# dongzhuoyao/self-guided-diffusion-models

Hardware: AMD Instinct MI355X
Metric: cfg_sampled_images_per_sec_64x64_1000step_ddpm (higher is better)
Workload: dtype f32 as 3xf16 split MFMA products, f32 accumulate; 1 GPU; IN64 unet_fast ch128 cluster-k5000 cond_scale=2 bs=40/GPU (UNet batch 80), 1000-step native DDPM; batch_per_gpu=40, unet_batch=80, precision_mode=f16x3, launch=hipGraph-captured step

## Files before the change

### include/sgdm_hip.h

```cpp
#ifndef SGDM_HIP_H
#define SGDM_HIP_H
#include <stdint.h>

#ifdef __cplusplus
extern "C" {
#endif

#define SGD_ABI_VERSION 24
int sgd_abi_version(void);
const char* sgd_build_id(void);

enum { SGD_MODE_FLAT = 0, SGD_MODE_CONV3 = 1 };
enum { SGD_RS_NONE = 0, SGD_RS_AVGPOOL2 = 1, SGD_RS_UP2 = 2,
       SGD_RS_ZEROUP2 = 3 ,
       SGD_RS_UP2_SUBPIXEL = 4 };
enum { SGD_PRO_NONE = 0, SGD_PRO_AFFINE_NC = 1, SGD_PRO_LN_ROW = 2 };
enum { SGD_PREC_F32 = 0, SGD_PREC_F16X3 = 1, SGD_PREC_BF16X3 = 2, SGD_PREC_F16 = 3, SGD_PREC_BF16 = 4 };

typedef struct sgd_igemm_args {
    const float* x0;
    const float* x1;
    int32_t c0, c1;
    int32_t mode;
    int32_t n, hi, wi;
// ... 21 lines not shown
    uint32_t drop_seed;
    float* stats;
    const float* w_scale_inv;
    void* work;
    int64_t work_bytes;
    int32_t grid_cap;
    int32_t tune;
} sgd_igemm_args;
enum {
    SGD_TUNE_BN128 = 1,
    SGD_TUNE_BN256 = 2,
    SGD_TUNE_FLAT2 = 4,
    SGD_TUNE_DEFER = 8,
    SGD_TUNE_PLAIN_SCHEDULE = 16,
    SGD_TUNE_NO_SMALL = 64,
    SGD_TUNE_LN_PACKED = 32,
    SGD_TUNE_WGRAD_GENERIC_NARROW = 256,
    SGD_TUNE_WGRAD_NO_POOLED_PLANES = 512,
    SGD_TUNE_WGRAD_F32 = 1024,
    SGD_TUNE_WGRAD_NO_WS = 2048,
    SGD_TUNE_WGRAD_NO_PLANES = 4096,
    SGD_TUNE_WGRAD_NO_PIPE = 8192,
    SGD_TUNE_WGRAD_PLANES_ALWAYS = 16384,
    SGD_TUNE_NO_SUBPIXEL = 32768
};
int64_t sgd_igemm_work_bytes(void);
int64_t sgd_igemm_work_status_offset(void);
int sgd_igemm_tail_layout(int32_t total_tiles, int32_t nchunks, int32_t taps, int32_t grid, int32_t* out);


int sgd_igemm(const sgd_igemm_args* args , void* stream);
int sgd_igemm_stats_parts(const sgd_igemm_args* args );
int sgd_igemm_subpixel_ok(const sgd_igemm_args* args );

int64_t sgd_packed_weight_bytes(int32_t cout, int32_t cin, int32_t ksize, int32_t prec);
int sgd_pack_weight(const float* w_src, void* w_dst, int32_t cout, int32_t cin, int32_t ksize,
                    int32_t prec, int32_t* cin_p, int32_t* cout_p , void* stream);

int64_t sgd_packed_weight_subpixel_bytes(int32_t cout, int32_t cin, int32_t prec);
int sgd_weight_amax_subpixel(const float* w_src, int32_t cout, int32_t cin, uint32_t* amax_bits, void* stream);
int sgd_pack_weight_subpixel_scaled(const float* w_src, void* w_dst, int32_t cout, int32_t cin, int32_t prec,
                                    const uint32_t* amax_bits, float* scale_inv_out, int32_t* cin_p, int32_t* cout_p ,
                                    void* stream);

int sgd_weight_amax(const float* w, int64_t count, uint32_t* amax_bits, void* stream);
int sgd_pack_weight_scaled(const float* w_src, void* w_dst, int32_t cout, int32_t cin, int32_t ksize, int32_t prec,
                           int32_t transpose ,
                           const uint32_t* amax_bits, float* scale_inv_out, int32_t* cin_p, int32_t* cout_p ,
// ... 228 lines not shown
```

### self-guided-diffusion-models_amd/csrc/igemm.hip

```cpp
#include <type_traits>
#include <utility>

#include "igemm_shared.h"
#include "prologue.h"

namespace {

#ifdef SGDM_PROBE
#define DBG(bit) 0
#define SYNC() do { if (g.stamp) { const unsigned long long t0_ = __builtin_amdgcn_s_memtime(); __syncthreads(); \
                    const unsigned long long t1_ = __builtin_amdgcn_s_memtime(); \
                    if (g.trace && blockIdx.x < 16 && pr_nbar < 512 && (threadIdx.x & 63) == 0) { \
                        unsigned long long* tp_ = g.trace + (((size_t)blockIdx.x * (NTHREADS / 64) + (threadIdx.x >> 6)) * 512 + pr_nbar) * 2; \
                        tp_[0] = t0_; tp_[1] = t1_; } \
                    pr_bar += t1_ - t0_; ++pr_nbar; } else if (!DBG(64)) { __syncthreads(); } } while (0)
#define PROBE_BEGIN() unsigned long long pr_bar = 0, pr_nbar = 0, pr_epi = 0; const unsigned long long pr_t0 = __builtin_amdgcn_s_memtime()
#define PROBE_END(role) do { if (g.stamp && (threadIdx.x & 63) == 0) { \
        unsigned long long* sp_ = g.stamp + ((size_t)blockIdx.x * (NTHREADS / 64) + (threadIdx.x >> 6)) * 4; \
        sp_[0] = __builtin_amdgcn_s_memtime() - pr_t0; sp_[1] = pr_bar; sp_[2] = pr_nbar; sp_[3] = pr_epi; } } while (0)
#define PROBE_EPI(expr) do { if (g.stamp) { const unsigned long long t0_ = __builtin_amdgcn_s_memtime(); expr; pr_epi += __builtin_amdgcn_s_memtime() - t0_; } else { expr; } } while (0)
#else
#define DBG(bit) 0
#define SYNC() __syncthreads()
#define PROBE_BEGIN()
// ... 248 lines not shown
    static constexpr int NA = 3;
    static constexpr int WM = (BN >= 128) ? 128 : 32;
    static constexpr int WN = (BN >= 128) ? BN / 4 : 32;
    static constexpr int MT = WM / 32, NT = WN / 32;
    static constexpr int WAVES_N = BN / WN;
    typedef Frag<PREC, NT> FragT;
    static constexpr bool M16 = PREC != SGD_PREC_F32 && BN <= 128 && !DEFER;
    static constexpr int RB = M16 ? WM / 16 : MT, RBH = M16 ? 16 : 32;
    static constexpr int CBN = M16 ? WN / 16 : NT, CBW = M16 ? 16 : 32;
    static constexpr int QPB = M16 ? 1 : 4;
    typedef Frag16<PREC, CBN> Frag16T;
    typedef std::conditional_t<M16, f32x4, f32x16> AccV;
    static constexpr int NKS = FragT::NKS;

    static constexpr int STG_LD = BN + 4;
    static_assert(!DEFER || (BN == 128 && TAPS == 9 && VEC && !M16), "loader-side epilogue: 3x3, 128-column tiles");
    static_assert(!SUBPIX || (VEC && PREC != SGD_PREC_F32 && BN >= 128), "sub-pixel conv: 16-byte inputs, split modes, 128-column tiles");

    const sgd_igemm_args& a;
    const Geo& g;
    float* As;
    int2* pixtab;
    float* bias_s;
    float* stg;
    int a_floats;
    bool bias_lds;
    int tid, lane, wave;
    int total, xchunk, nloc, xcd, loc, xbeg, xend, cin, nchunks, xtiles, nfull, xrem, split;
    int ntiles, rem_lin, rem_part, last_c0, last_c1;
    int Q, S, s, TW, TH, M;

    __device__ __forceinline__ int lin_of(int k) const { return (rem_lin >= 0 && k == ntiles - 1) ? rem_lin : xbeg + loc + k * nloc; }
    __device__ __forceinline__ int cbeg(int k) const { return k == ntiles - 1 ? last_c0 : 0; }
    __device__ __forceinline__ int cend(int k) const { return k == ntiles - 1 ? last_c1 : nchunks; }

    __device__ __forceinline__ bool init(float* smem) {
        a_floats = g.pix * LDA;
        As = smem;
        pixtab = reinterpret_cast<int2*>(smem + (size_t)NA * a_floats);
        bias_s = smem + (size_t)NA * a_floats + (size_t)g.pix * 8;
        bias_lds = a.cout_p <= BIAS_LDS_MAX;
        stg = bias_s + a.cout_p;

        tid = threadIdx.x; lane = tid & 63;
        wave = __builtin_amdgcn_readfirstlane(tid >> 6);

        total = g.mt * g.nt;
        xchunk = (total + 7) >> 3;
        nloc = gridDim.x >> 3;
// ... 70 lines not shown
        int px = l5;
        if (CONV && g.tw_l2 == 4 && s == 1) {
            if (l5 < 4) px = l5;
            else if (l5 < 12) px = l5 + 4;
            else if (l5 < 16) px = l5 - 8;
            else if (l5 < 20) px = l5;
            else if (l5 < 28) px = l5 + 2;
            else px = l5 < 30 ? l5 - 8 : l5;
        }
        if constexpr (M16) {
            const int i16 = ln & 15;
            px = i16 < 4 ? 2 * i16 : (i16 < 12 ? 2 * (i16 - 4) + 1 : 2 * i16 - 16);
        }
        return px;
    }
    template <int RES, bool PART>
    __device__ __forceinline__ void epilogue(const AccV (&acc)[RB][CBN], const Tile& T, int wm, int wn, int lane_e, int cb, float wsk,
                                             const char* part_base, int nparts) const;
    __device__ __forceinline__ void loader_role();
    __device__ __forceinline__ void compute_role();
};

template <int BN, int PREC, bool VEC, int TAPS, bool DEFER>
__device__ __forceinline__ void IgemmBlock<BN, PREC, VEC, TAPS, DEFER>::loader_role() {
    PROBE_BEGIN();
    __builtin_amdgcn_s_setprio(2);
    const int dlt = tid - NCOMP;
    const int dcq = (dlt >> 6) * 8 + (dlt & 7), drg = (dlt & 63) >> 3;
    int dk = 0, dqs = 0, dnck = cend(0) - cbeg(0);
    Tile dT = tile_at<SUBPIX>(g, lin_of(0), BN, TW, TH);
    int dcol = 0;
    unsigned dsoff = 0xFFFFFFFFu;
    f32x4 dres[8], ds1 = {0.f, 0.f, 0.f, 0.f}, ds2 = ds1;
// ... 67 lines not shown
            const Tile& T = dT;
#pragma unroll
            for (int jj = 0; jj < NQ; ++jj) {
                const int i = i0 + jj;
                const int row = drg + 8 * (i < 16 ? i : 15);
                const int tx = row & (TW - 1), ty = (row >> g.tw_l2) & (TH - 1), nb = row >> (g.tw_l2 + g.th_l2);
                const int n = T.img0 + nb;
                const bool ok = i < i1 && nb < g.nb && n < a.n && dcol < a.cout;
                const int orow = (n * a.ho + T.ty0 + ty) * a.wo + T.tx0 + tx;
                dyoff[jj] = ok ? (unsigned)(((long)orow * a.y_ld + dcol) * 4) : 0xFFFFFFFFu;
                const unsigned ro = ok ? (unsigned)(((long)orow * a.cout + dcol) * 4) : 0xFFFFFFFFu;
                dres[jj] = __builtin_bit_cast(f32x4, __builtin_amdgcn_raw_buffer_load_b128(dr_rs, ro, 0, 0));
            }
        }
        (void)q;
    };
    if constexpr (CONV) {
        const bool uni_rt = VEC && g.nb == 1 && a.pro == SGD_PRO_AFFINE_NC;
        const bool drop_rt = a.drop_p > 0.f;
        const bool lean2 = g.fast_a && VEC && ((uni_rt && a.pro_silu) || (a.pro == SGD_PRO_NONE && !a.pro_silu))
                           && (!drop_rt || (uni_rt && a.pro_silu && a.resample != SGD_RS_AVGPOOL2))
                           && cin % KC == 0 && (a.c1 == 0 || a.c0 % KC == 0) && !DBG(3);
        if (lean2) {
            constexpr int LT = A_THREADS;
            constexpr int AJ = (FAST_PIX * 8 + LT - 1) / LT;
            const int lt = tid - NCOMP;
            const int c4 = lt & 7;
            const int items = g.pix * 8;
            auto go = [&](auto unic, auto poolc, auto dropc) __attribute__((always_inline)) {
                constexpr bool uni = decltype(unic)::value;
// ... 95 lines not shown
#pragma unroll
                    for (int j = 0; j < AJ; ++j) issue_item(s2, j);
                };
                s2.k = 0; s2.chunk = cbeg(0); s2.img0 = tile_at<SUBPIX>(g, lin_of(0), BN, TW, TH).img0; fill(s2);
                load_rows(0);
                issue_coef(s2);
#pragma unroll
                for (int j = 0; j < AJ; ++j) issue_item(s2, j);
                stage(0);
                stage(1);
                SYNC();
                auto periods = [&](auto nqc) __attribute__((always_inline)) {
                    for (int q = 0; q < Q; ++q) {
                        drain(q, nqc);
                        stage((q + 2) % NA);
                        if (q + 4 < Q && (q + 4) % nchunks == 0) build_pixtab((q + 4) / nchunks, lt, LT);
                        SYNC();
                    }
                };
                if constexpr (NS == 4) periods(std::integral_constant<int, 0>());
                else with_nq(periods);
            };
            if (uni_rt) {
                if (a.resample == SGD_RS_AVGPOOL2) go(std::true_type(), std::true_type(), std::false_type());
                else if (drop_rt) go(std::true_type(), std::false_type(), std::true_type());
                else go(std::true_type(), std::false_type(), std::false_type());
            } else {
                if (a.resample == SGD_RS_AVGPOOL2) go(std::false_type(), std::true_type(), std::false_type());
                else go(std::false_type(), std::false_type(), std::false_type());
            }
            PROBE_END(1);
            return;
        }
// ... 235 lines not shown
                tr.tab = cx.tab;
                tr.m0 = 0;
#pragma unroll
                for (int j = 0; j < AJ; ++j)
                    finish_item(slot, tr, cx.chunk, lt + j * A_THREADS, araw[j], kshared, kq);
                cx = ctx_of(qnext);
                request();
            };
            request();
            stage(1, 2);
            SYNC();
            with_nq([&](auto nqc) __attribute__((always_inline)) {
                for (int q = 0; q < Q; ++q) {
                    drain(q, nqc);
                    stage(q + 2, q + 3);
                    if (q + 4 < Q && (q + 4) % nchunks == 0) build_pixtab((q + 4) / nchunks, lt, A_THREADS);
                    SYNC();
                }
            });
        } else {
            stage_A_sync(1, 1);
            SYNC();
            with_nq([&](auto nqc) __attribute__((always_inline)) {
                for (int q = 0; q < Q; ++q) {
                    drain(q, nqc);
                    stage_A_sync(q + 2, q + 2);
                    if (q + 4 < Q && (q + 4) % nchunks == 0) build_pixtab((q + 4) / nchunks, lt, A_THREADS);
                    SYNC();
                }
            });
        }
        PROBE_END(1);
        return;
    } else {
        constexpr int AJ = (BM * 8 + A_THREADS - 1) / A_THREADS;
        f32x4 araw[NB_RING][AJ];
        stage_A_sync(0, 0);
        if (Q > 1) stage_A_sync(1, 1);
        auto issue = [&](int q, auto rc) {
            constexpr int R = decltype(rc)::value;
            q = q < Q ? q : Q - 1;
            const int k = q / nchunks, chunk = q - k * nchunks + cbeg(k);
            const TabRef tab = tabref(k);
            const int c = chunk * KC + c4 * 4;
// ... 28 lines not shown
        for (; step + 3 <= S; step += 3) {
            body(step, R2());
            body(step + 1, R0());
            body(step + 2, R1());
        }
        if (step < S) {
            body(step, R2());
            if (step + 1 < S) body(step + 1, R0());
        }
        PROBE_END(1);
        return;
    }
}

template <int BN, int PREC, bool VEC, int TAPS, bool DEFER>
template <int RES, bool PART>
__device__ __forceinline__ void IgemmBlock<BN, PREC, VEC, TAPS, DEFER>::epilogue(const AccV (&acc)[RB][CBN], const Tile& T, int wm, int wn,
                                                                                 int lane_e, int cb, float wsk, const char* part_base,
                                                                                 int nparts) const {
    const int li = lane & 31;
    bool okm[RB];
    int orw[RB], rrw[RB];
    const int plie = pixel_of_lane(lane_e);
#pragma unroll
    for (int mt = 0; mt < RB; ++mt) {
        const int row = wm * WM + mt * RBH + plie;
        int orow, n = 0, oy = 0, ox = 0;
        if (CONV) {
            const int tx = row & (TW - 1), ty = (row >> g.tw_l2) & (TH - 1), nb = row >> (g.tw_l2 + g.th_l2);
            n = T.img0 + nb; oy = T.ty0 + ty; ox = T.tx0 + tx;
            okm[mt] = nb < g.nb && n < a.n;
// ... 18 lines not shown
    if (vec) {
        float* sp = nullptr;
        if (a.stats) {
            int n_img, part;
            if (CONV) {
                n_img = T.img0;
                part = ((T.par * g.tiles_y + (T.ty0 >> g.th_l2)) * g.tiles_x + (T.tx0 >> g.tw_l2)) * (BM / WM) + wm;
            } else {
                n_img = (int)(T.m0 / a.rows_per_n);
                part = (int)((T.m0 % a.rows_per_n) / BM) * (BM / WM) + wm;
            }
            sp = a.stats + ((long)n_img * g.sparts + part) * 2 * a.cout;
        }
        {
            constexpr int CS = CBN * QPB;
            constexpr int QB = M16 ? ((RES == 2 || PART) ? 1 : (CBN > 2 ? 2 : CBN)) : ((RES == 2 || NT > 1) ? 1 : 2);
            constexpr int RBB = M16 ? (RES == 2 || RB < 4 ? 2 : ((PART || CBN > 2) ? 4 : RB)) : RB;
            static_assert(RB % RBB == 0 && CS % QB == 0, "batches must tile the wave's rows and columns");
#pragma unroll
            for (int q0 = 0; q0 < CS; q0 += QB) {
            f32x4 s1[QB], s2[QB];
#pragma unroll
            for (int i = 0; i < QB; ++i) s1[i] = s2[i] = f32x4{0.f, 0.f, 0.f, 0.f};
#pragma unroll
            for (int mb0 = 0; mb0 < RB; mb0 += RBB) {
#pragma unroll
            for (int mt = mb0; mt < mb0 + RBB; ++mt) asm volatile("" : "+v"(orw[mt]), "+v"(rrw[mt]));
            f32x4 rv[QB][RBB];
            f32x4 pv[QB][RBB];
            if constexpr (PART) {
#pragma unroll
                for (int cs = q0; cs < q0 + QB; ++cs)
#pragma unroll
                    for (int mt = mb0; mt < mb0 + RBB; ++mt) {
                        const char* pp = part_base + (size_t)((mt * CS + cs) * NCOMP) * 16;
// ... 59 lines not shown
            }
        }
    } else {
#pragma unroll
        for (int mt = 0; mt < RB; ++mt) {
            if (!okm[mt]) continue;
            float* yp = a.y + (long)orw[mt] * a.y_ld;
            const float* rp = RES ? a.res + (long)rrw[mt] * a.cout : nullptr;
#pragma unroll
            for (int nt = 0; nt < CBN; ++nt)
#pragma unroll
                for (int gq = 0; gq < QPB; ++gq)
#pragma unroll
                    for (int j = 0; j < 4; ++j) {
                        const int c = cb + nt * CBW + gq * 8 + j;
                        if (c >= a.cout) continue;
                        float x = acc[mt][nt][(M16 ? 0 : gq * 4) + j];
                        if constexpr (PART) {
                            const float* pp = reinterpret_cast<const float*>(part_base + (size_t)(((mt * CBN + nt) * QPB + gq) * NCOMP) * 16) + j;
                            for (int pi = 0; pi < nparts; ++pi) x += pp[pi * (SLAB / 4)];
                        }
                        x = x * wsk + (bias_lds ? bias_s[c] : (a.bias ? a.bias[c] : 0.f));
                        if (RES == 1 || RES == 3) x += rp[c];
                        if (RES == 2) {
                            const long rw = (long)a.wo * 2 * a.cout;
                            x += 0.25f * (rp[c] + rp[a.cout + c] + rp[rw + c] + rp[rw + a.cout + c]);
                        }
                        yp[c] = x;
                    }
        }
// ... 88 lines not shown
                constexpr int P2 = nw < NM - P1 ? nw : NM - P1;
#pragma unroll
                for (int i = 0; i < P1; ++i) {
                    __builtin_amdgcn_sched_group_barrier(0x008, 1, 0);
                    __builtin_amdgcn_sched_group_barrier(0x100, 1, 0);
                }
#pragma unroll
                for (int i = 0; i < P2; ++i) {
                    __builtin_amdgcn_sched_group_barrier(0x008, 1, 0);
                    __builtin_amdgcn_sched_group_barrier(0x020, 1, 0);
                }
                if constexpr (NM - P1 - P2 > 0) __builtin_amdgcn_sched_group_barrier(0x008, NM - P1 - P2, 0);
            }
            __builtin_amdgcn_sched_barrier(0);
        });
        if constexpr (seam) SYNC();
    };

    auto wstart_of = [&](int k) { return wtile_of(k) + (size_t)cbeg(k) * TAPS * wstep; };
    const char* wp = wstart_of(0);
    if constexpr (M16) {
#pragma unroll
        for (int cb = 0; cb < CBN; ++cb) fb16[cb].load(wp + (cb >> 1) * wunit<PREC>() + (cb & 1) * 256);
    } else {
#pragma unroll
        for (int ks = 0; ks < NKS; ++ks) fb[ks].load(wp, ks);
    }
    SYNC();
    int pcur = par_off(0);
#pragma unroll
    for (int st = 0; st < (M16 ? RB : DEPTH); ++st) {
// ... 12 lines not shown
        const char* const wseam = k + 1 < ntiles ? wstart_of(k + 1) : nullptr;
        const int c_end = cend(k);
        const int pnext = k + 1 < ntiles ? par_off(k + 1) : pcur;
        for (int chunk = cbeg(k); chunk < c_end; ++chunk) {
            const int naslot = aslot + 1 == NA ? 0 : aslot + 1;
            const float* acur = As + (size_t)aslot * a_floats + pcur;
            const float* anext = As + (size_t)naslot * a_floats + (chunk + 1 == c_end ? pnext : pcur);
            const char* const wlast = chunk + 1 == c_end ? (wseam ? wseam : wp + (TAPS - 1) * wstep) : nullptr;
            static_for<TAPS>([&](auto tapc) {
                constexpr int tap = decltype(tapc)::value;
                const char* wnext = wp + wstep;
                if (tap + 1 == TAPS && wlast) wnext = wlast;
                do_step(acur, anext, tapc, std::integral_constant<int, tap & 1>(), wnext);
                wp = wnext;
            });
            aslot = naslot;
        }
        if constexpr (DEFER) {
            if (k + 1 < ntiles) {
                int plie = pli;
                asm volatile("" : "+v"(plie));
#pragma unroll
                for (int mt = 0; mt < RB; ++mt) {
                    float* sp = stg + (size_t)(wm * WM + mt * RBH + plie) * STG_LD + wn * WN + 4 * lh;
#pragma unroll
                    for (int q = 0; q < QPB; ++q) {
                        f32x4 v;
#pragma unroll
                        for (int j = 0; j < 4; ++j) v[j] = acc[mt][0][q * 4 + j];
                        *reinterpret_cast<f32x4*>(sp + q * 8) = v;
// ... 1 lines not shown
                }
                continue;
            }
        }

        const char* part_base = nullptr;
        int nparts = 0;
        float wsk = wsi;
        int* part_cnt = nullptr;
        if (rem_lin >= 0 && k == ntiles - 1) {
            const int gi = tail_counter(xcd, loc, nloc, split);
            int* const cnt = reinterpret_cast<int*>(a.work) + gi * 2;
            char* const slab0 = reinterpret_cast<char*>(a.work) + WORK_HEAD + (size_t)tail_slab(xcd, loc, nloc, split) * SLAB;
            if (rem_part + 1 < split) {
                __amdgpu_buffer_rsrc_t rs = __builtin_amdgcn_make_buffer_rsrc(slab0 + (size_t)rem_part * SLAB, 0, (int)SLAB, 0x00020000);
#pragma unroll
                for (int mt = 0; mt < RB; ++mt)
#pragma unroll
                    for (int nt = 0; nt < CBN; ++nt)
#pragma unroll
                        for (int q = 0; q < QPB; ++q)
                            __builtin_amdgcn_raw_buffer_store_b128(__builtin_bit_cast(u32x4_t, accq(acc, mt, nt, q)), rs,
                                                                   (((mt * CBN + nt) * QPB + q) * NCOMP + tid) * 16, 0, 16 );
                asm volatile("s_waitcnt vmcnt(0)" ::: "memory");
                if (lane == 0) __hip_atomic_fetch_add(cnt, 1, __ATOMIC_RELAXED, __HIP_MEMORY_SCOPE_AGENT);
                break;
            }
            int late = 0;
            if (lane == 0) {
                const int need = (split - 1) * (NCOMP / 64);
                int polls = 0;
                while (__hip_atomic_load(cnt, __ATOMIC_RELAXED, __HIP_MEMORY_SCOPE_AGENT) < need) {
                    __builtin_amdgcn_s_sleep(16);
                    if (++polls >= FINISH_POLL_MAX) { late = 1; break; }
                }
                int* const status = reinterpret_cast<int*>(a.work) + WORK_STATUS_INT;
                if (late) __hip_atomic_store(status, 1, __ATOMIC_RELAXED, __HIP_MEMORY_SCOPE_AGENT);
                else if (__hip_atomic_load(status, __ATOMIC_RELAXED, __HIP_MEMORY_SCOPE_AGENT) != 0) late = 2;
// ... 11 lines not shown
        }

        const Tile T = tile_at<SUBPIX>(g, lin_of(k), BN, TW, TH);
        int lane_e;
        asm volatile("v_mbcnt_lo_u32_b32 %0, -1, 0\n\tv_mbcnt_hi_u32_b32 %0, -1, %0" : "=v"(lane_e));
        const int cb = T.n0c + wn * WN + 4 * (M16 ? lane_e >> 4 : lane_e >> 5);
        auto keep_acc = [&]() {
#pragma unroll
            for (int i = 0; i < RB; ++i)
#pragma unroll
                for (int j = 0; j < CBN; ++j) KEEP_LIVE(acc[i][j]);
        };
        auto run_epilogue = [&](auto partc) {
            constexpr bool PARTV = decltype(partc)::value;
            if (DBG(16) || ABL(8)) keep_acc();
            else if (SUBPIX || !a.res) epilogue<0, PARTV>(acc, T, wm, wn, lane_e, cb, wsk, part_base, nparts);
            else if (a.res_mode == SGD_RS_NONE) epilogue<1, PARTV>(acc, T, wm, wn, lane_e, cb, wsk, part_base, nparts);
            else if (NT > 1) __builtin_trap();
            else if (a.res_mode == SGD_RS_AVGPOOL2) epilogue<2, PARTV>(acc, T, wm, wn, lane_e, cb, wsk, part_base, nparts);
            else epilogue<3, PARTV>(acc, T, wm, wn, lane_e, cb, wsk, part_base, nparts);
        };
        if (nparts) {
            run_epilogue(std::true_type());
            if (lane == 0) {
                if (__hip_atomic_fetch_add(part_cnt + 1, 1, __ATOMIC_RELAXED, __HIP_MEMORY_SCOPE_AGENT) == NCOMP / 64 - 1) {
                    __hip_atomic_store(part_cnt, 0, __ATOMIC_RELAXED, __HIP_MEMORY_SCOPE_AGENT);
                    __hip_atomic_store(part_cnt + 1, 0, __ATOMIC_RELAXED, __HIP_MEMORY_SCOPE_AGENT);
                }
            }
        } else {
// ... 126 lines not shown
```

### self-guided-diffusion-models_amd/csrc/igemm_host.hip

```cpp
#include <stdint.h>

#include "igemm_shared.h"

extern "C" int sgd_abi_version(void) { return SGD_ABI_VERSION; }

static inline int pick_bn(int cout) { return (cout % 128 == 0) ? 128 : 32; }

static inline int column_tile(const sgd_igemm_args& a) {
    const int bn = pick_bn(a.cout);
    if (bn != 128 || (a.tune & (SGD_TUNE_NO_SMALL | SGD_TUNE_BN128 | SGD_TUNE_BN256))) return bn;
    const long rows = a.mode == SGD_MODE_CONV3 ? (long)a.n * a.ho * a.wo : (long)a.m;
    const long t128 = ((rows + BM - 1) / BM) * ((a.cout + 127) / 128);
    return t128 * 4 <= device_cus() ? 32 : 128;
}

static int make_geo(const sgd_igemm_args& a, Geo& g, int bn, int& na, int fg = 1) {
    if (a.c0 <= 0 || a.c1 < 0 || a.cout <= 0 || a.y_ld < a.cout) return SGD_ERR_ARG;
    if (a.mode == SGD_MODE_CONV3) {
        if (a.n <= 0 || a.hi <= 0 || a.wi <= 0 || (a.stride != 1 && a.stride != 2)) return SGD_ERR_ARG;
        if (a.stride == 2 && a.resample != SGD_RS_NONE) return SGD_ERR_ARG;
        if (a.resample < SGD_RS_NONE || a.resample > SGD_RS_UP2_SUBPIXEL) return SGD_ERR_ARG;
        const bool sub = a.resample == SGD_RS_UP2_SUBPIXEL;
        const bool up = a.resample == SGD_RS_UP2 || a.resample == SGD_RS_ZEROUP2;
        g.hc = a.resample == SGD_RS_AVGPOOL2 ? a.hi / 2 : (up ? a.hi * 2 : a.hi);
// ... 101 lines not shown
    if ((a0.c0 & 3) || (a0.c1 & 3) || (a0.c1 > 0 && a0.c0 % KC != 0)) return false;
    if (column_tile(a0) != 128) return false;
    sgd_igemm_args a = a0;
    a.resample = SGD_RS_UP2_SUBPIXEL;
    Geo g;
    int na;
    if (make_geo(a, g, 128, na) != SGD_OK) return false;
    if (a.stats && g.sparts == 0) return false;
    const size_t smem = (size_t)na * g.pix * LDA * sizeof(float) + (size_t)g.pix * 32
                        + (a.cout <= BIAS_LDS_MAX ? (size_t)((a.cout + 127) / 128 * 128) * sizeof(float) : 0);
    return smem <= 160 * 1024;
}

extern "C" int sgd_igemm_subpixel_ok(const sgd_igemm_args* args) { return args && subpixel_ok(*args) ? 1 : 0; }

extern "C" int sgd_igemm(const sgd_igemm_args* args, void* stream) {
    SGD_CLEAR_ERR();
    if (!args) return SGD_ERR_ARG;
    KArgs ka;
    ka.a = *args;
    sgd_igemm_args& a = ka.a;
    Geo& g = ka.g;
    if (!a.x0 || !a.w || !a.y || a.c0 <= 0 || a.c1 < 0 || a.cout <= 0) return SGD_ERR_ARG;
    if (a.prec < SGD_PREC_F32 || a.prec > SGD_PREC_BF16) return SGD_ERR_ARG;
    if (a.c1 > 0 && (!a.x1 || a.c0 % KC != 0)) return SGD_ERR_ARG;
    if (a.y_ld < a.cout) return SGD_ERR_ARG;
    if (a.pro != SGD_PRO_NONE && (!a.pa || !a.pb)) return SGD_ERR_ARG;
    const int cin = a.c0 + a.c1;
    int bn = column_tile(a);
    if (a.cout_p % pick_bn(a.cout) != 0 || a.cout_p < a.cout || a.cin_p % KC != 0 || a.cin_p < cin) return SGD_ERR_ARG;
    const bool vec = (a.c0 % 4 == 0) && (a.c1 % 4 == 0);
    const bool conv = a.mode == SGD_MODE_CONV3;
    const bool sub = conv && a.resample == SGD_RS_UP2_SUBPIXEL;
    if (sub && !subpixel_ok(a)) return SGD_ERR_ARG;
// ... 19 lines not shown
        if (rows_out >= (1L << 31) || rows_res >= (1L << 31)) return SGD_ERR_ARG;
    }
#ifdef SGDM_PROBE
    {
        const char* e = getenv("SGDM_DBG");
        g.dbg = e ? atoi(e) : 0;
        const char* sp = getenv("SGDM_STAMP_PTR");
        g.stamp = sp ? reinterpret_cast<unsigned long long*>(strtoull(sp, nullptr, 0)) : nullptr;
        const char* tp = getenv("SGDM_TRACE_PTR");
        g.trace = tp ? reinterpret_cast<unsigned long long*>(strtoull(tp, nullptr, 0)) : nullptr;
    }
#endif
    const size_t smem = (size_t)na * g.pix * LDA * sizeof(float) + (size_t)g.pix * 32
                        + (a.cout_p <= BIAS_LDS_MAX ? (size_t)a.cout_p * sizeof(float) : 0);
    if (smem > 160 * 1024) return SGD_ERR_ARG;
    hipStream_t st = (hipStream_t)stream;
    int variant = vec ? 1 : 0;
    size_t smem_launch = smem;
    {
        const int nchunks = (cin + KC - 1) / KC;
        const long rows_out = (long)a.n * a.ho * a.wo;
        const size_t smem_defer = smem + (size_t)BM * (128 + 4) * sizeof(float);
        if (conv && vec && bn == 128 && a.prec != SGD_PREC_F32 && ((a.cout | a.y_ld) & 3) == 0
            && (!a.res || a.res_mode == SGD_RS_NONE) && a.resample != SGD_RS_AVGPOOL2 && a.cout_p <= BIAS_LDS_MAX && nchunks >= 3
            && rows_out * a.y_ld * 4 < (1L << 32) && (!a.stats || (long)a.n * g.sparts * 2 * a.cout * 4 < (1L << 32))
            && smem_defer <= 160 * 1024 && !sub && (a.tune & SGD_TUNE_DEFER)) {
            variant = 2;
            smem_launch = smem_defer;
        }
    }
    switch (a.prec) {
        case SGD_PREC_F32: return sgd_igemm_dispatch_f32(&ka, bn, variant, taps, smem_launch, st);
        case SGD_PREC_F16X3: return ln_nopk ? sgd_igemm_dispatch_f16x3_nopk(&ka, bn, variant, taps, smem_launch, st)
                                            : sgd_igemm_dispatch_f16x3(&ka, bn, variant, taps, smem_launch, st);
        case SGD_PREC_BF16X3: return ln_nopk ? sgd_igemm_dispatch_bf16x3_nopk(&ka, bn, variant, taps, smem_launch, st)
                                             : sgd_igemm_dispatch_bf16x3(&ka, bn, variant, taps, smem_launch, st);
        case SGD_PREC_F16: return ln_nopk ? sgd_igemm_dispatch_f16_nopk(&ka, bn, variant, taps, smem_launch, st)
                                          : sgd_igemm_dispatch_f16(&ka, bn, variant, taps, smem_launch, st);
        case SGD_PREC_BF16: return ln_nopk ? sgd_igemm_dispatch_bf16_nopk(&ka, bn, variant, taps, smem_launch, st)
                                           : sgd_igemm_dispatch_bf16(&ka, bn, variant, taps, smem_launch, st);
        default: return SGD_ERR_ARG;
    }
}
```

### self-guided-diffusion-models_amd/csrc/igemm_shared.h

```cpp
#pragma once
#include <stdlib.h>

#include "sgdm_common.h"
#include "../../include/sgdm_hip.h"

namespace {

constexpr int KC = 32;
constexpr int LDA = KC + 4;
constexpr int BM = 128;
constexpr int NB_RING = 3;
constexpr int BIAS_LDS_MAX = 4096;
constexpr int A_THREADS = 256;
constexpr int NCOMP = 256;
constexpr int NTHREADS = NCOMP + A_THREADS;
constexpr int WUNIT = 4096;
constexpr int MIN_PART_STEPS = 27;
constexpr int SPLIT_MAX = 4;
constexpr int WORK_TILES = 256;
constexpr int WORK_HEAD = WORK_TILES * 8;
constexpr int WORK_STATUS_INT = WORK_HEAD / 4 - 1;
constexpr int FINISH_POLL_MAX = 1 << 20;

__host__ __device__ inline int tail_split(int xrem, int nloc, int nchunks, int taps) {
// ... 7 lines not shown
__host__ __device__ inline int tail_slab(int xcd, int loc, int nloc, int split) {
    return xcd * ((nloc * 3) >> 2) + (loc / split) * (split - 1);
}
constexpr int FAST_PIX = 192;

struct Geo {
    int tw_l2, th_l2;
    int hh, hw;
    int nb;
    int tiles_x, tiles_y;
    int pix;
    int mt, nt;
    int hc, wc;
    int sparts;
    int fast_a;
#ifdef SGDM_PROBE
    int dbg;
    unsigned long long* stamp;
    unsigned long long* trace;
#endif
};

struct KArgs {
    sgd_igemm_args a;
    Geo g;
};

inline int ilog2(int v) { int l = 0; while ((1 << l) < v) ++l; return l; }
inline int device_cus() {
    static int cus = 0;
// ... 22 lines not shown
```

### self-guided-diffusion-models_amd/sgdm_amd/_lib.py

```python
import ctypes as C
import os

import torch

_HERE = os.path.dirname(os.path.abspath(__file__))
LIB_PATH = os.environ.get("SGDM_LIB_PATH") or os.path.join(_HERE, "lib", "libsgdm_hip.so")

MODE_FLAT, MODE_CONV3 = 0, 1
RS_NONE, RS_AVGPOOL2, RS_UP2, RS_ZEROUP2, RS_UP2_SUBPIXEL = 0, 1, 2, 3, 4
PRO_NONE, PRO_AFFINE_NC, PRO_LN_ROW = 0, 1, 2
PREC_F32, PREC_F16X3, PREC_BF16X3, PREC_F16, PREC_BF16 = 0, 1, 2, 3, 4
PREC_BY_NAME = {"f32": PREC_F32, "f16x3": PREC_F16X3, "bf16x3": PREC_BF16X3, "f16": PREC_F16, "bf16": PREC_BF16}
INFERENCE_ONLY = ("f16", "bf16")
ABI_VERSION = 24

TUNE_BN128, TUNE_BN256, TUNE_FLAT2, TUNE_DEFER, TUNE_PLAIN_SCHEDULE, TUNE_LN_PACKED, TUNE_NO_SMALL = 1, 2, 4, 8, 16, 32, 64
TUNE_WGRAD_GENERIC_NARROW, TUNE_WGRAD_NO_POOLED_PLANES, TUNE_WGRAD_F32 = 256, 512, 1024
TUNE_WGRAD_NO_WS, TUNE_WGRAD_NO_PLANES, TUNE_WGRAD_NO_PIPE, TUNE_WGRAD_PLANES_ALWAYS = 2048, 4096, 8192, 16384
TUNE_NO_SUBPIXEL = 32768
PACK_FORWARD, PACK_DGRAD, PACK_SUBPIXEL = 0, 1, 2

vp, i32, i64, f32 = C.c_void_p, C.c_int32, C.c_int64, C.c_float


class IgemmArgs(C.Structure):
    _fields_ = [
        ("x0", vp), ("x1", vp), ("c0", i32), ("c1", i32), ("mode", i32),
        ("n", i32), ("hi", i32), ("wi", i32), ("ho", i32), ("wo", i32), ("m", i32),
        ("rows_per_n", i32), ("stride", i32), ("resample", i32), ("pro", i32), ("pro_silu", i32),
        ("pa", vp), ("pb", vp), ("pc", vp), ("w", vp), ("cin_p", i32), ("cout_p", i32),
        ("bias", vp), ("res", vp), ("res_mode", i32), ("y", vp), ("cout", i32), ("y_ld", i32),
        ("orows_in", i32), ("orows_out", i32), ("orow_off", i32), ("prec", i32),
        ("drop_p", f32), ("drop_seed", C.c_uint32), ("stats", vp), ("w_scale_inv", vp),
        ("work", vp), ("work_bytes", i64), ("grid_cap", i32), ("tune", i32),
    ]


class PackJob(C.Structure):
    _fields_ = [("src", vp), ("dst", vp), ("amax_bits", vp), ("scale_inv", vp), ("cout", i32), ("cin", i32), ("ksize", i32),
                ("transpose", i32), ("own_amax", i32), ("reserved0", i32)]


SIGNATURES = {
    "sgd_abi_version": (i32, []),
    "sgd_build_id": (C.c_char_p, []),
    "sgd_igemm": (i32, [C.POINTER(IgemmArgs), vp]),
    "sgd_igemm_stats_parts": (i32, [C.POINTER(IgemmArgs)]),
    "sgd_igemm_subpixel_ok": (i32, [C.POINTER(IgemmArgs)]),
    "sgd_igemm_work_bytes": (i64, []),
    "sgd_igemm_work_status_offset": (i64, []),
    "sgd_igemm_tail_layout": (i32, [i32, i32, i32, i32, C.POINTER(i32)]),
    "sgd_stats_reduce": (i32, [vp, i32, i32, i32, vp, i32, i32, vp]),
    "sgd_packed_weight_bytes": (i64, [i32, i32, i32, i32]),
    "sgd_pack_weight": (i32, [vp, vp, i32, i32, i32, i32, C.POINTER(i32), C.POINTER(i32), vp]),
    "sgd_weight_amax": (i32, [vp, i64, vp, vp]),
    "sgd_pack_weight_scaled": (i32, [vp, vp, i32, i32, i32, i32, i32, vp, vp, C.POINTER(i32), C.POINTER(i32), vp]),
    "sgd_packed_weight_subpixel_bytes": (i64, [i32, i32, i32]),
    "sgd_weight_amax_subpixel": (i32, [vp, i32, i32, vp, vp]),
    "sgd_pack_weight_subpixel_scaled": (i32, [vp, vp, i32, i32, i32, vp, vp, C.POINTER(i32), C.POINTER(i32), vp]),
    "sgd_pack_job_blocks": (i32, [i32, i32, i32, i32, i32, C.POINTER(i32), C.POINTER(i32), C.POINTER(i32), C.POINTER(i32)]),
    "sgd_pack_weights_batched": (i32, [vp, i32, vp, vp, i32, vp, vp, i32, i32, vp]),
    "sgd_linear_splitk": (i32, [vp, i32, vp, vp, i32, i32, i32, vp, i32, vp, i32, vp]),
    "sgd_linear_splitk_t": (i32, [vp, i32, vp, i32, i32, i32, i32, vp, i32, vp, i32, vp]),
# ... 133 lines not shown
```

Before: 2.355 images/s.

## Split conv epilogue between compute and loader waves via LDS parking

For 3x3 conv implicit-GEMM tiles with 128 columns in split-precision mode, compute waves now park half of their accumulator columns in LDS at the end of a tile. Loader waves then run the epilogue for that half while compute waves handle the other half and move on to the next tile. The goal is to overlap epilogue cost with the next tile's main loop and shorten the compute-wave critical path. In exchange it needs extra LDS staging, which can lower occupancy, and adds a barrier after each chunk. It is gated by a host-side eligibility rule and can be disabled with a new tune flag.

```diff
diff --git a/include/sgdm_hip.h b/include/sgdm_hip.h
--- a/include/sgdm_hip.h
+++ b/include/sgdm_hip.h
@@ -59,6 +59,7 @@
     SGD_TUNE_DEFER = 8,
     SGD_TUNE_PLAIN_SCHEDULE = 16,
     SGD_TUNE_NO_SMALL = 64,
+    SGD_TUNE_NO_SPLIT_EPILOGUE = 128,
     SGD_TUNE_LN_PACKED = 32,
     SGD_TUNE_WGRAD_GENERIC_NARROW = 256,
     SGD_TUNE_WGRAD_NO_POOLED_PLANES = 512,
@@ -77,6 +78,7 @@
 int sgd_igemm(const sgd_igemm_args* args , void* stream);
 int sgd_igemm_stats_parts(const sgd_igemm_args* args );
 int sgd_igemm_subpixel_ok(const sgd_igemm_args* args );
+int sgd_igemm_split_epilogue_ok(const sgd_igemm_args* args );
 
 int64_t sgd_packed_weight_bytes(int32_t cout, int32_t cin, int32_t ksize, int32_t prec);
 int sgd_pack_weight(const float* w_src, void* w_dst, int32_t cout, int32_t cin, int32_t ksize,
diff --git a/self-guided-diffusion-models_amd/csrc/igemm.hip b/self-guided-diffusion-models_amd/csrc/igemm.hip
--- a/self-guided-diffusion-models_amd/csrc/igemm.hip
+++ b/self-guided-diffusion-models_amd/csrc/igemm.hip
@@ -286,6 +286,9 @@
     static constexpr int NKS = FragT::NKS;
 
     static constexpr int STG_LD = BN + 4;
+    static constexpr bool SPLITC = M16 && BN == 128 && CONV && VEC;
+    static constexpr int CSH = CBN * QPB / 2;
+    static constexpr int HQ = RB * (CBN / 2) * (M16 ? 1 : 4);
     static_assert(!DEFER || (BN == 128 && TAPS == 9 && VEC && !M16), "loader-side epilogue: 3x3, 128-column tiles");
     static_assert(!SUBPIX || (VEC && PREC != SGD_PREC_F32 && BN >= 128), "sub-pixel conv: 16-byte inputs, split modes, 128-column tiles");
 
@@ -305,6 +308,9 @@
     __device__ __forceinline__ int lin_of(int k) const { return (rem_lin >= 0 && k == ntiles - 1) ? rem_lin : xbeg + loc + k * nloc; }
     __device__ __forceinline__ int cbeg(int k) const { return k == ntiles - 1 ? last_c0 : 0; }
     __device__ __forceinline__ int cend(int k) const { return k == ntiles - 1 ? last_c1 : nchunks; }
+    __device__ __forceinline__ bool split_tile(int k) const {
+        return SPLITC && !ABL(8) && g.split_epi && !(rem_lin >= 0 && k == ntiles - 1);
+    }
 
     __device__ __forceinline__ bool init(float* smem) {
         a_floats = g.pix * LDA;
@@ -405,9 +411,62 @@
         }
         return px;
     }
-    template <int RES, bool PART>
+    template <int RES, bool PART, int CS0 = 0, int CSN = -1>
     __device__ __forceinline__ void epilogue(const AccV (&acc)[RB][CBN], const Tile& T, int wm, int wn, int lane_e, int cb, float wsk,
                                              const char* part_base, int nparts) const;
+    __device__ __forceinline__ void park_half(const AccV (&acc)[RB][CBN], int w) const {
+        f32x4* hp = reinterpret_cast<f32x4*>(stg) + (size_t)w * HQ * 64 + lane;
+        int i = 0;
+#pragma unroll
+        for (int mt = 0; mt < RB; ++mt)
+#pragma unroll
+            for (int nt = CBN / 2; nt < CBN; ++nt)
+#pragma unroll
+                for (int q = 0; q < QPB; ++q) hp[(i++) * 64] = accq(acc, mt, nt, q);
+    }
+    __device__ __forceinline__ void loader_half(int k) const {
+        if constexpr (SPLITC) {
+            auto kp4 = __builtin_amdgcn_kernarg_segment_ptr();
+            asm volatile("" : "+s"(kp4));
+            const KArgs* kp = (const KArgs*)kp4;
+            IgemmBlock hb{kp->a, kp->g};
+            hb.bias_s = bias_s; hb.bias_lds = bias_lds; hb.stg = stg; hb.lane = lane; hb.wave = wave; hb.tid = tid;
+            hb.s = s; hb.TW = TW; hb.TH = TH; hb.M = M;
+            hb.ntiles = ntiles; hb.rem_lin = rem_lin; hb.xbeg = xbeg; hb.loc = loc; hb.nloc = nloc;
+            hb.half_body(k);
+        }
+        (void)k;
+    }
+    __device__ __forceinline__ void half_body(int k) const {
+        {
+            const int w = wave - NCOMP / 64;
+            const f32x4* hp = reinterpret_cast<const f32x4*>(stg) + (size_t)w * HQ * 64 + lane;
+            AccV acc[RB][CBN];
+            int i = 0;
+#pragma unroll
+            for (int mt = 0; mt < RB; ++mt)
+#pragma unroll
+                for (int nt = CBN / 2; nt < CBN; ++nt)
+#pragma unroll
+                    for (int q = 0; q < QPB; ++q) {
+                        const f32x4 v = hp[(i++) * 64];
+#pragma unroll
+                        for (int j = 0; j < 4; ++j) acc[mt][nt][(M16 ? 0 : q * 4) + j] = v[j];
+                    }
+#pragma unroll
+            for (int mt = 0; mt < RB; ++mt)
+#pragma unroll
+                for (int nt = 0; nt < CBN / 2; ++nt) acc[mt][nt] = AccV{};
+            const Tile T = tile_at<SUBPIX>(g, lin_of(k), BN, TW, TH);
+            const int wm = w / WAVES_N, wn = w % WAVES_N;
+            const int cb = T.n0c + wn * WN + 4 * (M16 ? lane >> 4 : lane >> 5);
+            const float wsi = a.w_scale_inv ? *a.w_scale_inv : 1.f;
+            constexpr int CS = CBN * QPB;
+            if (SUBPIX || !a.res) epilogue<0, false, CSH, CS - CSH>(acc, T, wm, wn, lane, cb, wsi, nullptr, 0);
+            else epilogue<1, false, CSH, CS - CSH>(acc, T, wm, wn, lane, cb, wsi, nullptr, 0);
+        }
+        (void)k;
+    }
     __device__ __forceinline__ void loader_role();
     __device__ __forceinline__ void compute_role();
 };
@@ -505,6 +564,22 @@
             }
         }
         (void)q;
+    };
+    int hk = 0, hq = SPLITC ? cend(0) - cbeg(0) : 0;
+    auto half_hook = [&](int q) __attribute__((always_inline)) {
+        if constexpr (SPLITC) {
+            if (q == hq) {
+                if (split_tile(hk)) loader_half(hk);
+                ++hk;
+                hq += cend(hk) - cbeg(hk);
+            }
+        }
+        (void)q;
+    };
+    auto half_last = [&]() __attribute__((always_inline)) {
+        if constexpr (SPLITC) {
+            if (split_tile(ntiles - 1)) loader_half(ntiles - 1);
+        }
     };
     if constexpr (CONV) {
         const bool uni_rt = VEC && g.nb == 1 && a.pro == SGD_PRO_AFFINE_NC;
@@ -630,9 +705,11 @@
                     for (int q = 0; q < Q; ++q) {
                         drain(q, nqc);
                         stage((q + 2) % NA);
+                        if constexpr (NS == 1) half_hook(q);
                         if (q + 4 < Q && (q + 4) % nchunks == 0) build_pixtab((q + 4) / nchunks, lt, LT);
                         SYNC();
                     }
+                    if constexpr (NS == 1) half_last();
                 };
                 if constexpr (NS == 4) periods(std::integral_constant<int, 0>());
                 else with_nq(periods);
@@ -898,9 +975,11 @@
                 for (int q = 0; q < Q; ++q) {
                     drain(q, nqc);
                     stage(q + 2, q + 3);
+                    half_hook(q);
                     if (q + 4 < Q && (q + 4) % nchunks == 0) build_pixtab((q + 4) / nchunks, lt, A_THREADS);
                     SYNC();
                 }
+                half_last();
             });
         } else {
             stage_A_sync(1, 1);
@@ -909,9 +988,11 @@
                 for (int q = 0; q < Q; ++q) {
                     drain(q, nqc);
                     stage_A_sync(q + 2, q + 2);
+                    half_hook(q);
                     if (q + 4 < Q && (q + 4) % nchunks == 0) build_pixtab((q + 4) / nchunks, lt, A_THREADS);
                     SYNC();
                 }
+                half_last();
             });
         }
         PROBE_END(1);
@@ -970,7 +1051,7 @@
 }
 
 template <int BN, int PREC, bool VEC, int TAPS, bool DEFER>
-template <int RES, bool PART>
+template <int RES, bool PART, int CS0, int CSN>
 __device__ __forceinline__ void IgemmBlock<BN, PREC, VEC, TAPS, DEFER>::epilogue(const AccV (&acc)[RB][CBN], const Tile& T, int wm, int wn,
                                                                                  int lane_e, int cb, float wsk, const char* part_base,
                                                                                  int nparts) const {
@@ -1019,11 +1100,13 @@
         }
         {
             constexpr int CS = CBN * QPB;
-            constexpr int QB = M16 ? ((RES == 2 || PART) ? 1 : (CBN > 2 ? 2 : CBN)) : ((RES == 2 || NT > 1) ? 1 : 2);
+            constexpr int CSE = CSN < 0 ? CS : CS0 + CSN;
+            constexpr int QBW = M16 ? ((RES == 2 || PART) ? 1 : (CBN > 2 ? 2 : CBN)) : ((RES == 2 || NT > 1) ? 1 : 2);
+            constexpr int QB = QBW < CSE - CS0 ? QBW : CSE - CS0;
             constexpr int RBB = M16 ? (RES == 2 || RB < 4 ? 2 : ((PART || CBN > 2) ? 4 : RB)) : RB;
-            static_assert(RB % RBB == 0 && CS % QB == 0, "batches must tile the wave's rows and columns");
-#pragma unroll
-            for (int q0 = 0; q0 < CS; q0 += QB) {
+            static_assert(RB % RBB == 0 && (CSE - CS0) % QB == 0 && CSE <= CS, "batches must tile the wave's rows and columns");
+#pragma unroll
+            for (int q0 = CS0; q0 < CSE; q0 += QB) {
             f32x4 s1[QB], s2[QB];
 #pragma unroll
             for (int i = 0; i < QB; ++i) s1[i] = s2[i] = f32x4{0.f, 0.f, 0.f, 0.f};
@@ -1113,6 +1196,7 @@
 #pragma unroll
                     for (int j = 0; j < 4; ++j) {
                         const int c = cb + nt * CBW + gq * 8 + j;
+                        if (CSN >= 0 && (nt * QPB + gq < CS0 || nt * QPB + gq >= CS0 + CSN)) continue;
                         if (c >= a.cout) continue;
                         float x = acc[mt][nt][(M16 ? 0 : gq * 4) + j];
                         if constexpr (PART) {
@@ -1231,7 +1315,7 @@
             }
             __builtin_amdgcn_sched_barrier(0);
         });
-        if constexpr (seam) SYNC();
+        if constexpr (seam && !SPLITC) SYNC();
     };
 
     auto wstart_of = [&](int k) { return wtile_of(k) + (size_t)cbeg(k) * TAPS * wstep; };
@@ -1274,6 +1358,10 @@
                 do_step(acur, anext, tapc, std::integral_constant<int, tap & 1>(), wnext);
                 wp = wnext;
             });
+            if constexpr (SPLITC) {
+                if (chunk + 1 == c_end && split_tile(k)) park_half(acc, wave);
+                SYNC();
+            }
             aslot = naslot;
         }
         if constexpr (DEFER) {
@@ -1305,6 +1393,9 @@
             char* const slab0 = reinterpret_cast<char*>(a.work) + WORK_HEAD + (size_t)tail_slab(xcd, loc, nloc, split) * SLAB;
             if (rem_part + 1 < split) {
                 __amdgpu_buffer_rsrc_t rs = __builtin_amdgcn_make_buffer_rsrc(slab0 + (size_t)rem_part * SLAB, 0, (int)SLAB, 0x00020000);
+                int lane_s;
+                asm volatile("v_mbcnt_lo_u32_b32 %0, -1, 0\n\tv_mbcnt_hi_u32_b32 %0, -1, %0" : "=v"(lane_s));
+                const int tid_s = wave * 64 + lane_s;
 #pragma unroll
                 for (int mt = 0; mt < RB; ++mt)
 #pragma unroll
@@ -1312,7 +1403,7 @@
 #pragma unroll
                         for (int q = 0; q < QPB; ++q)
                             __builtin_amdgcn_raw_buffer_store_b128(__builtin_bit_cast(u32x4_t, accq(acc, mt, nt, q)), rs,
-                                                                   (((mt * CBN + nt) * QPB + q) * NCOMP + tid) * 16, 0, 16 );
+                                                                   (((mt * CBN + nt) * QPB + q) * NCOMP + tid_s) * 16, 0, 16 );
                 asm volatile("s_waitcnt vmcnt(0)" ::: "memory");
                 if (lane == 0) __hip_atomic_fetch_add(cnt, 1, __ATOMIC_RELAXED, __HIP_MEMORY_SCOPE_AGENT);
                 break;
@@ -1354,6 +1445,12 @@
         auto run_epilogue = [&](auto partc) {
             constexpr bool PARTV = decltype(partc)::value;
             if (DBG(16) || ABL(8)) keep_acc();
+            else if (!PARTV && split_tile(k)) {
+                if constexpr (SPLITC) {
+                    if (SUBPIX || !a.res) epilogue<0, false, 0, CSH>(acc, T, wm, wn, lane_e, cb, wsk, part_base, nparts);
+                    else epilogue<1, false, 0, CSH>(acc, T, wm, wn, lane_e, cb, wsk, part_base, nparts);
+                }
+            }
             else if (SUBPIX || !a.res) epilogue<0, PARTV>(acc, T, wm, wn, lane_e, cb, wsk, part_base, nparts);
             else if (a.res_mode == SGD_RS_NONE) epilogue<1, PARTV>(acc, T, wm, wn, lane_e, cb, wsk, part_base, nparts);
             else if (NT > 1) __builtin_trap();
diff --git a/self-guided-diffusion-models_amd/csrc/igemm_host.hip b/self-guided-diffusion-models_amd/csrc/igemm_host.hip
--- a/self-guided-diffusion-models_amd/csrc/igemm_host.hip
+++ b/self-guided-diffusion-models_amd/csrc/igemm_host.hip
@@ -139,10 +139,22 @@
 
 extern "C" int sgd_igemm_subpixel_ok(const sgd_igemm_args* args) { return args && subpixel_ok(*args) ? 1 : 0; }
 
-extern "C" int sgd_igemm(const sgd_igemm_args* args, void* stream) {
-    SGD_CLEAR_ERR();
+static bool split_epilogue_rule(const sgd_igemm_args& a, int bn, int variant, int nchunks, size_t smem, size_t* stg_bytes) {
+    const size_t stg = (size_t)4 * 64 * (BM * (bn / 4) / 64 / 2) * sizeof(float);
+    if (stg_bytes) *stg_bytes = stg;
+    if (a.tune & SGD_TUNE_NO_SPLIT_EPILOGUE) return false;
+    if (a.mode != SGD_MODE_CONV3 || bn != 128 || a.prec == SGD_PREC_F32 || variant != 1) return false;
+    if (((a.cout | a.y_ld) & 3) != 0) return false;
+    if (a.res && a.res_mode != SGD_RS_NONE) return false;
+    if (a.resample == SGD_RS_AVGPOOL2) return false;
+    if (a.cout_p > BIAS_LDS_MAX || nchunks < 2) return false;
+    return smem + stg <= 160 * 1024;
+}
+
+struct Plan { int bn, variant, taps; size_t smem; bool ln_nopk; };
+
+static int plan_igemm(const sgd_igemm_args* args, KArgs& ka, Plan& pl) {
     if (!args) return SGD_ERR_ARG;
-    KArgs ka;
     ka.a = *args;
     sgd_igemm_args& a = ka.a;
     Geo& g = ka.g;
@@ -192,7 +204,6 @@
     const size_t smem = (size_t)na * g.pix * LDA * sizeof(float) + (size_t)g.pix * 32
                         + (a.cout_p <= BIAS_LDS_MAX ? (size_t)a.cout_p * sizeof(float) : 0);
     if (smem > 160 * 1024) return SGD_ERR_ARG;
-    hipStream_t st = (hipStream_t)stream;
     int variant = vec ? 1 : 0;
     size_t smem_launch = smem;
     {
@@ -206,7 +217,33 @@
             variant = 2;
             smem_launch = smem_defer;
         }
-    }
+        size_t stg_bytes = 0;
+        g.split_epi = split_epilogue_rule(a, bn, variant, nchunks, smem, &stg_bytes) ? 1 : 0;
+        if (g.split_epi) smem_launch = smem + stg_bytes;
+    }
+    pl.bn = bn; pl.variant = variant; pl.taps = taps; pl.smem = smem_launch; pl.ln_nopk = ln_nopk;
+    return SGD_OK;
+}
+
+extern "C" int sgd_igemm_split_epilogue_ok(const sgd_igemm_args* args) {
+    KArgs ka;
+    Plan pl;
+    return plan_igemm(args, ka, pl) == SGD_OK && ka.g.split_epi ? 1 : 0;
+}
+
+extern "C" int sgd_igemm(const sgd_igemm_args* args, void* stream) {
+    SGD_CLEAR_ERR();
+    KArgs ka;
+    Plan pl;
+    {
+        const int rc = plan_igemm(args, ka, pl);
+        if (rc != SGD_OK) return rc;
+    }
+    const sgd_igemm_args& a = ka.a;
+    const int bn = pl.bn, variant = pl.variant, taps = pl.taps;
+    const size_t smem_launch = pl.smem;
+    const bool ln_nopk = pl.ln_nopk;
+    hipStream_t st = (hipStream_t)stream;
     switch (a.prec) {
         case SGD_PREC_F32: return sgd_igemm_dispatch_f32(&ka, bn, variant, taps, smem_launch, st);
         case SGD_PREC_F16X3: return ln_nopk ? sgd_igemm_dispatch_f16x3_nopk(&ka, bn, variant, taps, smem_launch, st)
diff --git a/self-guided-diffusion-models_amd/csrc/igemm_shared.h b/self-guided-diffusion-models_amd/csrc/igemm_shared.h
--- a/self-guided-diffusion-models_amd/csrc/igemm_shared.h
+++ b/self-guided-diffusion-models_amd/csrc/igemm_shared.h
@@ -45,6 +45,7 @@
     int hc, wc;
     int sparts;
     int fast_a;
+    int split_epi;
 #ifdef SGDM_PROBE
     int dbg;
     unsigned long long* stamp;
diff --git a/self-guided-diffusion-models_amd/sgdm_amd/_lib.py b/self-guided-diffusion-models_amd/sgdm_amd/_lib.py
--- a/self-guided-diffusion-models_amd/sgdm_amd/_lib.py
+++ b/self-guided-diffusion-models_amd/sgdm_amd/_lib.py
@@ -18,6 +18,7 @@
 TUNE_WGRAD_GENERIC_NARROW, TUNE_WGRAD_NO_POOLED_PLANES, TUNE_WGRAD_F32 = 256, 512, 1024
 TUNE_WGRAD_NO_WS, TUNE_WGRAD_NO_PLANES, TUNE_WGRAD_NO_PIPE, TUNE_WGRAD_PLANES_ALWAYS = 2048, 4096, 8192, 16384
 TUNE_NO_SUBPIXEL = 32768
+TUNE_NO_SPLIT_EPILOGUE = 128
 PACK_FORWARD, PACK_DGRAD, PACK_SUBPIXEL = 0, 1, 2
 
 vp, i32, i64, f32 = C.c_void_p, C.c_int32, C.c_int64, C.c_float
@@ -47,6 +48,7 @@
     "sgd_igemm": (i32, [C.POINTER(IgemmArgs), vp]),
     "sgd_igemm_stats_parts": (i32, [C.POINTER(IgemmArgs)]),
     "sgd_igemm_subpixel_ok": (i32, [C.POINTER(IgemmArgs)]),
+    "sgd_igemm_split_epilogue_ok": (i32, [C.POINTER(IgemmArgs)]),
     "sgd_igemm_work_bytes": (i64, []),
     "sgd_igemm_work_status_offset": (i64, []),
     "sgd_igemm_tail_layout": (i32, [i32, i32, i32, i32, C.POINTER(i32)]),
```

Result: no change. 2.368 images/s, median of 6 (+0.5%).
